# HSoumi/hybrid-als-twotower-recommender

Measured on NVIDIA B200. Metric: als_ratings_per_sec_per_sweep, higher is better.
Workload: dtype f32

## Files before the change

hybrid-als-twotower-recommender_b200/csrc/als_tc_common.cuh:

```cuda
#pragma once
#include <cuda_bf16.h>
#include <stdint.h>

#include "als_prep.cuh"
#include "common.cuh"

namespace hals {

__device__ __forceinline__ float4 lds128(uint32_t addr) {
  float4 v;
  asm volatile("ld.shared.v4.f32 {%0,%1,%2,%3}, [%4];\n" : "=f"(v.x), "=f"(v.y), "=f"(v.z), "=f"(v.w) : "r"(addr));
  return v;
}
__device__ __forceinline__ float lds32(uint32_t addr) {
  float v;
  asm volatile("ld.shared.f32 %0, [%1];\n" : "=f"(v) : "r"(addr));
  return v;
}
__device__ __forceinline__ void sts128(uint32_t addr, float a, float b, float c, float d) {
  asm volatile("st.shared.v4.f32 [%0], {%1,%2,%3,%4};\n" ::"r"(addr), "f"(a), "f"(b), "f"(c), "f"(d) : "memory");
}
__device__ __forceinline__ void sts32(uint32_t addr, float a) {
  asm volatile("st.shared.f32 [%0], %1;\n" ::"r"(addr), "f"(a) : "memory");
}

typedef unsigned long long f32x2;
__device__ __forceinline__ f32x2 pack2(float lo, float hi) {
  f32x2 r;
  asm("mov.b64 %0, {%1, %2};\n" : "=l"(r) : "f"(lo), "f"(hi));
  return r;
}
__device__ __forceinline__ float lo2(f32x2 v) { return __uint_as_float((uint32_t)v); }
__device__ __forceinline__ float hi2(f32x2 v) { return __uint_as_float((uint32_t)(v >> 32)); }
__device__ __forceinline__ f32x2 ffma2(f32x2 a, f32x2 b, f32x2 c) {
  f32x2 d;
  asm("fma.rn.f32x2 %0, %1, %2, %3;\n" : "=l"(d) : "l"(a), "l"(b), "l"(c));
  return d;
}
__device__ __forceinline__ void lds128x2(uint32_t addr, f32x2& p0, f32x2& p1) {
  asm volatile("ld.shared.v2.b64 {%0,%1}, [%2];\n" : "=l"(p0), "=l"(p1) : "r"(addr));
}
__device__ __forceinline__ f32x2 lds64x2(uint32_t addr) {
  f32x2 p;
  asm volatile("ld.shared.b64 %0, [%1];\n" : "=l"(p) : "r"(addr));
  return p;
}
__device__ __forceinline__ void sts128x2(uint32_t addr, f32x2 p0, f32x2 p1) {
  asm volatile("st.shared.v2.b64 [%0], {%1,%2};\n" ::"r"(addr), "l"(p0), "l"(p1) : "memory");
}

__device__ __forceinline__ void sts128x2_if(bool pred, uint32_t addr, f32x2 p0, f32x2 p1) {
  asm volatile("{\n\t.reg .pred p;\n\tsetp.ne.b32 p, %3, 0;\n\t@p st.shared.v2.b64 [%0], {%1,%2};\n\t}\n"
               ::"r"(addr), "l"(p0), "l"(p1), "r"((uint32_t)pred) : "memory");
}
__device__ __forceinline__ void sts32_if(bool pred, uint32_t addr, float a) {
  asm volatile("{\n\t.reg .pred p;\n\tsetp.ne.b32 p, %2, 0;\n\t@p st.shared.f32 [%0], %1;\n\t}\n"
               ::"r"(addr), "f"(a), "r"((uint32_t)pred) : "memory");
}

__device__ __forceinline__ void bar_sync_64(int id) { asm volatile("bar.sync %0, 64;\n" ::"r"(id) : "memory"); }


__device__ __forceinline__ void bar_arrive_n(int id, int nthreads) {
  asm volatile("bar.arrive %0, %1;\n" ::"r"(id), "r"(nthreads) : "memory");
}
__device__ __forceinline__ void bar_sync_n(int id, int nthreads) {
  asm volatile("bar.sync %0, %1;\n" ::"r"(id), "r"(nthreads) : "memory");
}

int als_launch_reduce_solve128(const float* slots, float* dst, float reg, const hals_als_plan* plan, void* dst_hl,
                               const float* gram, cudaStream_t st);

}
```

hybrid-als-twotower-recommender_b200/csrc/als_ws64.cu:

```cuda
#include <cuda_bf16.h>

#include <cstdlib>

#include "als_ws_common.cuh"

namespace hals {
namespace ws64 {
using namespace ws;

constexpr int K = 64;
constexpr int kStageBytes = stage_bytes(K);
#ifndef HALS_WS_STAGES
#define HALS_WS_STAGES 10
#endif
constexpr int kStages = HALS_WS_STAGES;
constexpr int kAcc = 4, kAccCols = 128;
constexpr int kSlots = 2;
constexpr int kLd = 68;
constexpr int kSlotBytes = 2 * 64 * kLd * 4 + 512;
constexpr int kSolvers = 9;
constexpr int kScratchBytes = 1536;
constexpr int kN = 80;
constexpr int kThreads = 512;
constexpr int kWarpSolver = 0, kWarpGather = 9, kWarpMma = 11, kWarpDrain = 12;
static_assert(kStages % 2 == 0, "the two gather warps own alternate stages");
static_assert(kWarpSolver + kSolvers == kWarpGather && kWarpDrain + 4 == kThreads / 32 && kWarpDrain % 4 == 0, "role map");

struct Bars {
  uint64_t st_full[kStages], st_free[kStages];
  uint64_t st_scaled[kStages];
  uint64_t acc_full[kAcc], acc_free[kAcc];
  uint64_t sol_full[kSolvers];
  uint64_t slot_free[kSlots];
};

__device__ __forceinline__ float sel4(float a, float b, float c, float d, int i) {
  return i == 0 ? a : i == 1 ? b : i == 2 ? c : d;
}

__device__ __noinline__ void gather_role(uint32_t stages, Bars* bars, uint8_t* gscratch, const Range* rg,
                                         const int32_t* __restrict__ colidx, const uint32_t* __restrict__ vals_hl,
                                         const float* __restrict__ vals_sc, const uint8_t* __restrict__ src_hl, int zero_row,
                                         const int64_t* __restrict__ chunk_pos, const int32_t* __restrict__ chunk_cnt,
                                         int gw, int lane) {
  const int t_sub = lane >> 4, piece = lane & 15;
  const uint32_t ring = umma::smem_u32(gscratch);
  const uint32_t mpos = ring + 2 * kBurst * 128;
  const uint32_t mcnt = mpos + 2 * kBurst * 8;
  const int64_t k_hi = rg->chunk_hi;
  int64_t kw = rg->chunk_lo + gw;
  auto load_window = [&](int64_t& p, int& c) {
    const int64_t k = kw + 2 * lane;
    p = 0; c = 0;
    if (k < k_hi) { p = __ldg(chunk_pos + k); c = __ldg(chunk_cnt + k); }
    kw += 64;
  };
  int64_t wpos, npos;
  int wcnt, ncnt;
  load_window(wpos, wcnt);
  load_window(npos, ncnt);
  int wb = 0;
  int ci[kBurst];
  auto fill = [&](int buf) {
    if (lane >= wb * kBurst && lane < (wb + 1) * kBurst) {
      const uint32_t e = (uint32_t)(buf * kBurst + lane - wb * kBurst);
      asm volatile("st.shared.b64 [%0], %1;\n" ::"r"(mpos + e * 8u), "l"(wpos) : "memory");
      asm volatile("st.shared.b32 [%0], %1;\n" ::"r"(mcnt + e * 4u), "r"(wcnt) : "memory");
    }
#pragma unroll
    for (int c = 0; c < kBurst; ++c) {
      const int64_t pos = __shfl_sync(0xffffffffu, wpos, wb * kBurst + c);
      const int cnt = __shfl_sync(0xffffffffu, wcnt, wb * kBurst + c);
      ci[c] = lane < cnt ? __ldg(colidx + pos + lane) : zero_row;
    }
    if (++wb == 32 / kBurst) {
      wb = 0;
      wpos = npos; wcnt = ncnt;
      load_window(npos, ncnt);
    }
  };
  auto stash = [&](int buf) {
#pragma unroll
    for (int c = 0; c < kBurst; ++c)
      sts32(ring + (uint32_t)((buf * kBurst + c) * 32 + (lane & 1) * 16 + (lane >> 1)) * 4u, __int_as_float(ci[c]));
    __syncwarp();
  };

  const uint32_t blk_off = piece < 8 ? 0u : (uint32_t)kBlk;
  uint32_t dsto[4];
#pragma unroll
  for (int i = 0; i < 4; ++i) {
    const int t = t_sub + 2 * i;
    dsto[i] = blk_off + (uint32_t)t * kRowBytes + (uint32_t)(((piece & 7) ^ (t & 7)) << 4);
  }
  const uint64_t srcb = reinterpret_cast<uint64_t>(src_hl) + (uint64_t)piece * 16u;
  const uint32_t rdst = 2 * kBlk + (uint32_t)lane * kRowBytes + (uint32_t)((lane & 7) << 4);
  const uint32_t sdst = 2 * kBlk + (uint32_t)lane * kRowBytes + (uint32_t)((7 ^ (lane & 7)) << 4);
  uint32_t g = 0, s = (uint32_t)gw, u = 0;
#ifdef HALS_WS_PROFILE
  long long w_free = 0, t_iss = 0, t_fill = 0;
#endif
  fill(0);
  stash(0);
  fill(1);
  for (int buf = 0;; buf ^= 1) {
    bool done = false;
#pragma unroll 1
    for (int c = 0; c < kBurst; ++c) {
      int cnt;
      asm volatile("ld.shared.b32 %0, [%1];\n" : "=r"(cnt) : "r"(mcnt + (uint32_t)(buf * kBurst + c) * 4u));
      if (cnt <= 0) { done = true; break; }
      int64_t pos;
      asm volatile("ld.shared.b64 %0, [%1];\n" : "=l"(pos) : "r"(mpos + (uint32_t)(buf * kBurst + c) * 8u));
      const uint32_t ir = ring + (uint32_t)((buf * kBurst + c) * 32 + t_sub * 16) * 4u;
      const float4 c0 = lds128(ir), c1 = lds128(ir + 16), c2 = lds128(ir + 32), c3 = lds128(ir + 48);
      if (u > 0) { WS_T0(); umma::mbar_wait(&bars->st_free[s], (u - 1) & 1); WS_ACC(w_free); }
      WS_T0();
      const uint32_t st = stages + s * kStageBytes;
      const float colf[16] = {c0.x, c0.y, c0.z, c0.w, c1.x, c1.y, c1.z, c1.w, c2.x, c2.y, c2.z, c2.w, c3.x, c3.y, c3.z, c3.w};
#pragma unroll
      for (int i = 0; i < KC / 2; ++i) {
        uint64_t src;
        asm("mad.wide.u32 %0, %1, 256, %2;\n" : "=l"(src) : "r"((uint32_t)__float_as_int(colf[i])), "l"(srcb));
        cp_async16_raw(st + dsto[i & 3] + (uint32_t)(i >> 2) * (8 * kRowBytes), src);
      }
      {
        const bool ok = lane < cnt;
        const uint32_t* rp = vals_hl + pos + (ok ? lane : 0);
        asm volatile("cp.async.ca.shared.global [%0], [%1], 4, %2;\n" ::"r"(st + rdst), "l"(rp), "r"(ok ? 4 : 0) : "memory");
        if (vals_sc != nullptr) {
          const float* sp = vals_sc + pos + (ok ? lane : 0);
          asm volatile("cp.async.ca.shared.global [%0], [%1], 4, %2;\n" ::"r"(st + sdst), "l"(sp), "r"(ok ? 4 : 0) : "memory");
        }
      }
      cp_async_mbar_arrive_noinc(&bars->st_full[s]);
      WS_ACC(t_iss);
      ++g;
      s += 2;
      if (s >= (uint32_t)kStages) { s -= kStages; ++u; }
    }
    if (done) break;
    WS_T0();
    stash(buf ^ 1);
    fill(buf);
    WS_ACC(t_fill);
  }
#ifdef HALS_WS_PROFILE
  if (lane == 0 && blockIdx.x == 1) printf("G%d: chunks %u wait_free %lld issue %lld fill %lld\n", gw, g, w_free, t_iss, t_fill);
#endif
}

__device__ __noinline__ void scaler_role(uint32_t stages, Bars* bars, const Range* rg, int lane) {
  scale_stages<K, kStages>(stages, bars, rg, lane);
}

__device__ __noinline__ void mma_role(uint32_t sbase, uint32_t tmem, Bars* bars, const Range* rg,
                                      const int32_t* __restrict__ chunk_cnt, bool scaled, int lane) {
  constexpr uint32_t idesc = umma::make_instr_desc(umma::kFmtBF16, true, true, 128, kN);
  uint64_t* const ready = scaled ? bars->st_scaled : bars->st_full;
  const int64_t k_lo = rg->chunk_lo, k_hi = rg->chunk_hi;
  uint32_t s = 0, su = 0, b = 0, bu = 0;
  bool first = true;
#ifdef HALS_WS_PROFILE
  long long w_acc = 0, w_full = 0, t_issue = 0;
#endif
  int wc = 0, nc = 0;
  if (k_lo + lane < k_hi) wc = __ldg(chunk_cnt + k_lo + lane);
  if (k_lo + 32 + lane < k_hi) nc = __ldg(chunk_cnt + k_lo + 32 + lane);
  const bool leader = elect_one();
  const uint64_t ad0 = umma::make_smem_desc(sbase, kBlk, 1024, umma::kSwizzle128B);
  const uint64_t bd0 = umma::make_smem_desc(sbase, 2 * kBlk, 1024, umma::kSwizzle128B);
  for (int64_t kb = k_lo; kb < k_hi; kb += 32) {
    const int nk = (int)(k_hi - kb < 32 ? k_hi - kb : 32);
    for (int i = 0; i < nk; ++i) {
      const int cnt = __shfl_sync(0xffffffffu, wc, i);
      if (leader) {
        if (first) {
          if (bu > 0) { WS_T0(); umma::mbar_wait(&bars->acc_free[b], (bu - 1) & 1); WS_ACC(w_acc); }
          umma::fence_after_sync();
        }
        { WS_T0(); umma::mbar_wait(&ready[s], su & 1); WS_ACC(w_full); }
        WS_T0();
        const uint32_t td = tmem + b * kAccCols;
        const uint64_t so = (uint64_t)((s * kStageBytes) >> 4);
#pragma unroll
        for (int ks = 0; ks < KC / 16; ++ks)
          umma::mma_bf16(td, ad0 + so + (uint64_t)(ks * 2048 >> 4), bd0 + so + (uint64_t)(ks * 2048 >> 4), idesc,
                         !(first && ks == 0));
        umma::commit(&bars->st_free[s]);
        if (cnt <= KC) umma::commit(&bars->acc_full[b]);
        WS_ACC(t_issue);
      }
      __syncwarp();
      first = cnt <= KC;
      if (first) { if (++b == (uint32_t)kAcc) { b = 0; ++bu; } }
      if (++s == (uint32_t)kStages) { s = 0; ++su; }
    }
    wc = nc;
    nc = 0;
    if (kb + 64 + lane < k_hi) nc = __ldg(chunk_cnt + kb + 64 + lane);
  }
#ifdef HALS_WS_PROFILE
  if (blockIdx.x == 1 && leader) printf("M: wait_acc_free %lld wait_stage_full %lld issue %lld\n", w_acc, w_full, t_issue);
#endif
}

__device__ __noinline__ void drain_role(uint32_t slots, uint32_t tmem, Bars* bars, const Range* rg, int nsolv, int tid) {
  const int warp = tid >> 5;
  const int64_t n_rows = rg->item_hi - rg->item_lo;
  uint32_t b = 0, bu = 0, sl = 0, slu = 0, sv = 0;
#ifdef HALS_WS_PROFILE
  long long w_acc = 0, w_slot = 0, t_ld = 0;
#endif
  for (int64_t it = 0; it < n_rows; ++it) {
    { WS_T0(); umma::mbar_wait(&bars->acc_full[b], bu & 1); WS_ACC(w_acc); }
    umma::fence_after_sync();
    const uint32_t ta = tmem + b * kAccCols + ((uint32_t)(warp * 32) << 16);
    float a[64], e[16];
    {
      WS_T0();
      umma::tmem_ld32(ta, a);
      umma::tmem_ld32(ta + 32, a + 32);
      umma::tmem_ld16(ta + 64, e);
      WS_ACC(t_ld);
    }
    umma::fence_before_sync();
    umma::mbar_arrive(&bars->acc_free[b]);
    if (slu > 0) { WS_T0(); umma::mbar_wait(&bars->slot_free[sl], (slu - 1) & 1); WS_ACC(w_slot); }
    const uint32_t sb = slots + sl * kSlotBytes;
    const int m = tid & 63;
    const uint32_t rowp = sb + (tid < 64 ? 0u : (uint32_t)(64 * kLd * 4)) + (uint32_t)m * (kLd * 4);
#pragma unroll
    for (int n = 0; n < 64; n += 4) sts128(rowp + n * 4, a[n], a[n + 1], a[n + 2], a[n + 3]);
    const uint32_t bp = sb + 2 * 64 * kLd * 4;
    if (tid < 64) sts32(bp + m * 4, e[0] + e[1]);
    else sts32(bp + 256 + m * 4, e[0]);
    umma::mbar_arrive(&bars->sol_full[sv]);
    if (++b == (uint32_t)kAcc) { b = 0; ++bu; }
    if (++sl == (uint32_t)kSlots) { sl = 0; ++slu; }
    if (++sv == (uint32_t)nsolv) sv = 0;
  }
#ifdef HALS_WS_PROFILE
  if (tid == 0 && blockIdx.x == 1) printf("D: wait_acc_full %lld tmem_ld %lld wait_slot_free %lld\n", w_acc, t_ld, w_slot);
#endif
}

template <int JR>
__device__ __forceinline__ void elim_block(f32x2 (&R)[36], f32x2& bb2, const uint32_t P, const uint32_t Y,
                                           const uint32_t DI, const int ti, const int tj, const int lane) {
  const uint32_t oW = (uint32_t)ti * 16u;
  const uint32_t oL = (uint32_t)(tj & 3) * 16u + (uint32_t)(tj >> 2) * 4u;
  const uint32_t oB = oW + (uint32_t)(tj >> 1) * 64u + (uint32_t)(tj & 1) * 8u;
  auto publish = [&](uint32_t Pn, bool own) {
    if (JR & 1) sts64_if(own, Pn + oW + (JR >> 1) * 64 + 8, R[tri(JR, JR)]);
#pragma unroll
    for (int q = (JR + 1) & ~1; q < 8; q += 2) sts128x2_if(own, Pn + oW + (q >> 1) * 64, R[tri(q, JR)], R[tri(q + 1, JR)]);
  };
  {
    publish(P, tj == 0);
    sts32_if(ti == 0 && tj == JR, Y + (uint32_t)(8 * JR) * 4u, lo2(bb2));
    sts32_if(lane == 0, DI + (uint32_t)(8 * JR) * 4u, -rcp_fast(lo2(R[tri(JR, JR)])));
    __syncwarp();
  }
  const bool below = tj > JR;
#pragma unroll 1
  for (int jm = 0; jm < 8; ++jm) {
    const int j = 8 * JR + jm;
    const uint32_t Pj = P + ((uint32_t)(jm & 1) << 8);
    f32x2 w[8];
    float l[8];
    if (JR & 1) w[JR] = lds64x2(Pj + oW + (JR >> 1) * 64 + 8);
#pragma unroll
    for (int q = (JR + 1) & ~1; q < 8; q += 2) lds128x2(Pj + oW + (q >> 1) * 64, w[q], w[q + 1]);
    const float ninv = lds32(DI + (uint32_t)j * 4u);
#pragma unroll
    for (int c = JR; c < 8; ++c) l[c] = lds32(Pj + oL + (c >> 1) * 64 + (c & 1) * 8);
    const float zj = lds32(Y + (uint32_t)j * 4u);
    const f32x2 wb = lds64x2(Pj + oB);
    const f32x2 ninv2 = pack2(ninv, ninv);
    const float lj = tj > jm ? l[JR] : 0.f;
    const f32x2 lj2 = pack2(lj, lj);
    w[JR] = fmul2(w[JR], ninv2);
    R[tri(JR, JR)] = ffma2(w[JR], lj2, R[tri(JR, JR)]);
    const int jn = jm + 1;
    const float ninv_n = -rcp_fast((jn & 4) ? hi2(R[tri(JR, JR)]) : lo2(R[tri(JR, JR)]));
#pragma unroll
    for (int q = JR + 1; q < 8; ++q) {
      w[q] = fmul2(w[q], ninv2);
      R[tri(q, JR)] = ffma2(w[q], lj2, R[tri(q, JR)]);
    }
    {
      const bool on = tj == JR;
      const bool act_lo = below || (on && ti > jm), act_hi = below || (on && ti + 4 > jm);
      const f32x2 mb = fmul2(wb, ninv2);
      bb2 = ffma2(pack2(act_lo ? lo2(mb) : 0.f, act_hi ? hi2(mb) : 0.f), pack2(zj, zj), bb2);
    }
    {
      const uint32_t Pn = P + ((uint32_t)(jn & 1) << 8);
      const bool own = (tj == jn);
      publish(Pn, own);
      sts32_if(tj == JR && ti == (jn & 3) && jn < 8, Y + (uint32_t)(j + 1) * 4u, (jn & 4) ? hi2(bb2) : lo2(bb2));
      sts32_if(own && ti == (jn & 3), DI + (uint32_t)(j + 1) * 4u, ninv_n);
      __syncwarp();
    }
#pragma unroll
    for (int c = JR + 1; c < 8; ++c) {
      const f32x2 l2 = pack2(l[c], l[c]);
#pragma unroll
      for (int q = c; q < 8; ++q) R[tri(q, c)] = ffma2(w[q], l2, R[tri(q, c)]);
    }
  }
}

template <int JR>
__device__ __forceinline__ void back_block(const f32x2 (&R)[36], f32x2 (&x2)[8], const uint32_t Y, const uint32_t DI,
                                           const uint32_t T, const uint32_t RH, const int ti, const int tj,
                                           const int lane, float& out0, float& out1) {
  f32x2 acc0 = 0ull, acc1 = 0ull;
#pragma unroll
  for (int q = JR + 1; q < 8; ++q) {
    if ((q - JR) & 1) acc0 = ffma2(R[tri(q, JR)], x2[q], acc0);
    else acc1 = ffma2(R[tri(q, JR)], x2[q], acc1);
  }
  float ext = (lo2(acc0) + hi2(acc0)) + (lo2(acc1) + hi2(acc1));
  ext += __shfl_xor_sync(0xffffffffu, ext, 8);
  ext += __shfl_xor_sync(0xffffffffu, ext, 16);
  const float rh = lds32(Y + (uint32_t)(8 * JR + tj) * 4u) - ext;
  sts32(T + (uint32_t)(ti * 8 + tj) * 4u, lo2(R[tri(JR, JR)]));
  sts32(T + (uint32_t)((ti + 4) * 8 + tj) * 4u, hi2(R[tri(JR, JR)]));
  sts32_if(ti == 0, RH + (uint32_t)tj * 4u, rh);
  __syncwarp();
  float r[8], di[8], xb[8];
  {
    const float4 a = lds128(RH), b = lds128(RH + 16);
    r[0] = a.x; r[1] = a.y; r[2] = a.z; r[3] = a.w; r[4] = b.x; r[5] = b.y; r[6] = b.z; r[7] = b.w;
    const float4 c = lds128(DI + (uint32_t)(8 * JR) * 4u), d = lds128(DI + (uint32_t)(8 * JR) * 4u + 16);
    di[0] = c.x; di[1] = c.y; di[2] = c.z; di[3] = c.w; di[4] = d.x; di[5] = d.y; di[6] = d.z; di[7] = d.w;
  }
#pragma unroll
  for (int e = 7; e >= 0; --e) {
    xb[e] = -r[e] * di[e];
    if (e > 0) {
      float t[8];
      const float4 a = lds128(T + (uint32_t)(e * 8) * 4u);
      t[0] = a.x; t[1] = a.y; t[2] = a.z; t[3] = a.w;
      if (e > 4) {
        const float4 b = lds128(T + (uint32_t)(e * 8 + 4) * 4u);
        t[4] = b.x; t[5] = b.y; t[6] = b.z; t[7] = b.w;
      }
#pragma unroll
      for (int c = 0; c < e; ++c) r[c] = fmaf(-t[c], xb[e], r[c]);
    }
  }
  __syncwarp();
  x2[JR] = pack2(sel4(xb[0], xb[1], xb[2], xb[3], ti), sel4(xb[4], xb[5], xb[6], xb[7], ti));
  if ((lane >> 2) == JR) {
    const int e2 = lane & 3;
    out0 = sel4(xb[0], xb[2], xb[4], xb[6], e2);
    out1 = sel4(xb[1], xb[3], xb[5], xb[7], e2);
  }
}

__device__ __forceinline__ void eliminate(f32x2 (&R)[36], f32x2& bb2, const uint32_t P, const uint32_t Y, const uint32_t DI,
                                          int ti, int tj, int lane) {
  elim_block<0>(R, bb2, P, Y, DI, ti, tj, lane);
  elim_block<1>(R, bb2, P, Y, DI, ti, tj, lane);
  elim_block<2>(R, bb2, P, Y, DI, ti, tj, lane);
  elim_block<3>(R, bb2, P, Y, DI, ti, tj, lane);
  elim_block<4>(R, bb2, P, Y, DI, ti, tj, lane);
  elim_block<5>(R, bb2, P, Y, DI, ti, tj, lane);
  elim_block<6>(R, bb2, P, Y, DI, ti, tj, lane);
  elim_block<7>(R, bb2, P, Y, DI, ti, tj, lane);
  __syncwarp();
}
__device__ __forceinline__ void back_store(const f32x2 (&R)[36], const uint32_t Y, const uint32_t DI, const uint32_t T,
                                           const uint32_t RH, int ti, int tj, int lane, float* __restrict__ dst,
                                           __nv_bfloat16* __restrict__ dst_hl, int row) {
  f32x2 x2[8];
#pragma unroll
  for (int q = 0; q < 8; ++q) x2[q] = 0ull;
  float out0 = 0.f, out1 = 0.f;
  back_block<7>(R, x2, Y, DI, T, RH, ti, tj, lane, out0, out1);
  back_block<6>(R, x2, Y, DI, T, RH, ti, tj, lane, out0, out1);
  back_block<5>(R, x2, Y, DI, T, RH, ti, tj, lane, out0, out1);
  back_block<4>(R, x2, Y, DI, T, RH, ti, tj, lane, out0, out1);
  back_block<3>(R, x2, Y, DI, T, RH, ti, tj, lane, out0, out1);
  back_block<2>(R, x2, Y, DI, T, RH, ti, tj, lane, out0, out1);
  back_block<1>(R, x2, Y, DI, T, RH, ti, tj, lane, out0, out1);
  back_block<0>(R, x2, Y, DI, T, RH, ti, tj, lane, out0, out1);
  *reinterpret_cast<float2*>(dst + (int64_t)row * K + 2 * lane) = make_float2(out0, out1);
  if (dst_hl) {
    const __nv_bfloat162 h = __floats2bfloat162_rn(out0, out1);
    const __nv_bfloat162 l = __floats2bfloat162_rn(out0 - __low2float(h), out1 - __high2float(h));
    __nv_bfloat162* o = reinterpret_cast<__nv_bfloat162*>(dst_hl + (int64_t)row * (2 * K));
    o[lane] = h;
    o[K / 2 + lane] = l;
  }
}

__device__ __noinline__ void solver_role(uint32_t slots, uint32_t scratch, Bars* bars, float* __restrict__ dst,
                                         __nv_bfloat16* __restrict__ dst_hl, float* __restrict__ workspace, float reg,
                                         const int32_t* __restrict__ item_row, const int32_t* __restrict__ item_len,
                                         const int32_t* __restrict__ item_slot, const float* __restrict__ gram_tiles,
                                         const Range* rg, int nsolv, int w, int lane) {
  const int ti = lane >> 3, tj = lane & 7;
  const uint32_t P = scratch, Y = P + 512, DI = Y + 256, T = DI + 256, RH = T + 256;
  const int64_t n_items = rg->item_hi;
#ifdef HALS_WS_PROFILE
  long long w_slot = 0, t_load = 0, t_elim = 0, t_back = 0;
  int n_solved = 0;
#endif
  int64_t it = rg->item_lo + w;
  int row_n = 0, len_n = 0, slot_n = -1;
  if (it < n_items) { row_n = __ldg(item_row + it); len_n = __ldg(item_len + it); slot_n = __ldg(item_slot + it); }
  uint32_t mine = 0;
  for (uint32_t i = (uint32_t)w; it < n_items; i += nsolv, it += nsolv, ++mine) {
    const int row = row_n, len = len_n, wslot = slot_n;
    {
      const int64_t nx = it + nsolv;
      if (nx < n_items) { row_n = __ldg(item_row + nx); len_n = __ldg(item_len + nx); slot_n = __ldg(item_slot + nx); }
    }
    const uint32_t sl = i % kSlots;
    { WS_T0(); umma::mbar_wait(&bars->sol_full[w], mine & 1); WS_ACC(w_slot); }
    const uint32_t S1 = slots + sl * kSlotBytes, S2 = S1 + 64 * kLd * 4, B1 = S2 + 64 * kLd * 4, B2 = B1 + 256;
    if (wslot >= 0) {
      float* W = workspace + (size_t)wslot * ((size_t)K * K + K + 4);
      for (int e = lane; e < K * K; e += 32) {
        const int m = e >> 6, n = e & 63;
        W[e] = lds32(S1 + (uint32_t)(m * kLd + n) * 4u) + lds32(S2 + (uint32_t)(m * kLd + n) * 4u) +
               lds32(S2 + (uint32_t)(n * kLd + m) * 4u);
      }
      W[K * K + lane] = lds32(B1 + lane * 4) + lds32(B2 + lane * 4);
      W[K * K + 32 + lane] = lds32(B1 + (32 + lane) * 4) + lds32(B2 + (32 + lane) * 4);
      if (lane == 0) W[K * K + K] = (float)len;
      __syncwarp();
      if (lane == 0) umma::mbar_arrive(&bars->slot_free[sl]);
      continue;
    }
    f32x2 R[36];
    f32x2 bb2;
    {
      WS_T0();
      const float lam = reg * (float)len;
      const uint32_t p1 = S1 + (uint32_t)(ti * kLd + tj) * 4u, p2 = S2 + (uint32_t)(ti * kLd + tj) * 4u;
      const uint32_t pt = S2 + (uint32_t)(tj * kLd + ti) * 4u;
#pragma unroll
      for (int q = 0; q < 8; ++q) {
#pragma unroll
        for (int c = 0; c <= q; ++c) {
          float v[2];
#pragma unroll
          for (int h = 0; h < 2; ++h) {
            const uint32_t mn = (uint32_t)((8 * q + 4 * h) * kLd + 8 * c) * 4u, nm = (uint32_t)(8 * c * kLd + 8 * q + 4 * h) * 4u;
            v[h] = lds32(p1 + mn) + lds32(p2 + mn) + lds32(pt + nm);
            if (q == c) v[h] += (ti + 4 * h == tj) ? lam : 0.f;
          }
          R[tri(q, c)] = pack2(v[0], v[1]);
        }
      }
      if (gram_tiles != nullptr) {
        const float4* gp = reinterpret_cast<const float4*>(gram_tiles) + lane * 18;
#pragma unroll
        for (int i = 0; i < 18; ++i) {
          const float4 g = __ldg(gp + i);
          R[2 * i] = ffma2(pack2(g.x, g.y), pack2(1.f, 1.f), R[2 * i]);
          R[2 * i + 1] = ffma2(pack2(g.z, g.w), pack2(1.f, 1.f), R[2 * i + 1]);
        }
      }
      const uint32_t ob = (uint32_t)(ti + 8 * tj) * 4u;
      bb2 = pack2(lds32(B1 + ob) + lds32(B2 + ob), lds32(B1 + ob + 16) + lds32(B2 + ob + 16));
      __syncwarp();
      if (lane == 0) umma::mbar_arrive(&bars->slot_free[sl]);
      WS_ACC(t_load);
    }
    {
      WS_T0();
      eliminate(R, bb2, P, Y, DI, ti, tj, lane);
      WS_ACC(t_elim);
    }
    {
      WS_T0();
      back_store(R, Y, DI, T, RH, ti, tj, lane, dst, dst_hl, row);
      WS_ACC(t_back);
    }
#ifdef HALS_WS_PROFILE
    ++n_solved;
#endif
  }
#ifdef HALS_WS_PROFILE
  if (lane == 0 && blockIdx.x == 1)
    printf("S%d: solved %d wait_slot %lld load %lld elim %lld back %lld\n", w, n_solved, w_slot, t_load, t_elim, t_back);
#endif
}

__global__ void __launch_bounds__(kThreads, 1)
als_ws64_kernel(const int32_t* __restrict__ colidx, const uint32_t* __restrict__ vals_hl,
                const float* __restrict__ vals_sc, const float* __restrict__ gram_tiles,
                const __nv_bfloat16* __restrict__ src_hl, float* __restrict__ dst, float reg,
                const int32_t* __restrict__ item_row, const int32_t* __restrict__ item_len,
                const int32_t* __restrict__ item_slot, const int64_t* __restrict__ item_chunk0,
                const int64_t* __restrict__ item_cost0, const int64_t* __restrict__ chunk_pos,
                const int32_t* __restrict__ chunk_cnt, int64_t n_items, int zero_row, float* __restrict__ workspace,
                __nv_bfloat16* __restrict__ dst_hl) {
  extern __shared__ uint8_t smem_dyn[];
  __shared__ Bars bars;
  __shared__ Range range;
  __shared__ uint32_t tmem_slot;
  uint8_t* base = reinterpret_cast<uint8_t*>((reinterpret_cast<uintptr_t>(smem_dyn) + 1023) & ~uintptr_t(1023));
  const int tid = threadIdx.x, warp = tid >> 5, lane = tid & 31;
  if (warp == kWarpDrain) umma::tmem_alloc(&tmem_slot, kAcc * kAccCols);
  if (tid == 32) {
    for (int s = 0; s < kStages; ++s) {
      umma::mbar_init(&bars.st_full[s], 32);
      umma::mbar_init(&bars.st_free[s], 1);
      umma::mbar_init(&bars.st_scaled[s], 1);
    }
    for (int b = 0; b < kAcc; ++b) { umma::mbar_init(&bars.acc_full[b], 1); umma::mbar_init(&bars.acc_free[b], 128); }
    for (int s = 0; s < kSlots; ++s) umma::mbar_init(&bars.slot_free[s], 1);
    for (int s = 0; s < kSolvers; ++s) umma::mbar_init(&bars.sol_full[s], 128);
    umma::mbar_fence_init();
  }
  if (tid < 2) cta_range(&range, item_cost0, item_chunk0, n_items, tid);
  zero_r_blocks<K, kStages, kThreads>(base, tid);
  umma::fence_proxy_async();
  umma::fence_before_sync();
  __syncthreads();
  umma::fence_after_sync();
  const uint32_t tmem = tmem_slot;
  const uint32_t sbase = umma::smem_u32(base);
#ifdef HALS_WS_PROFILE
  const long long t_cta0 = clock64();
#endif
  const uint32_t slots = sbase + kStages * kStageBytes;
  const uint32_t scratch = slots + kSlots * kSlotBytes;
  uint8_t* gscratch = base + kStages * kStageBytes + kSlots * kSlotBytes + kSolvers * kScratchBytes;

  const bool implicit = vals_sc != nullptr;
  const int nsolv = implicit ? kSolvers - 1 : kSolvers;
  if (warp >= kWarpDrain) {
    drain_role(slots, tmem, &bars, &range, nsolv, tid - kWarpDrain * 32);
  } else if (warp >= kWarpGather && warp < kWarpMma) {
    gather_role(sbase, &bars, gscratch + (warp - kWarpGather) * kGatherScratch, &range, colidx, vals_hl, vals_sc,
                reinterpret_cast<const uint8_t*>(src_hl), zero_row, chunk_pos, chunk_cnt, warp - kWarpGather, lane);
  } else if (warp == kWarpMma) {
    mma_role(sbase, tmem, &bars, &range, chunk_cnt, implicit, lane);
  } else if (warp - kWarpSolver < nsolv) {
    solver_role(slots, scratch + (uint32_t)(warp - kWarpSolver) * kScratchBytes, &bars, dst, dst_hl, workspace, reg, item_row,
                item_len, item_slot, gram_tiles, &range, nsolv, warp - kWarpSolver, lane);
  } else {
    scaler_role(sbase, &bars, &range, lane);
  }
#ifdef HALS_WS_PROFILE
  const long long t_role = clock64() - t_cta0;
#endif
  umma::fence_before_sync();
  __syncthreads();
#ifdef HALS_WS_PROFILE
  if (lane == 0 && (warp == kWarpDrain || warp == kWarpGather || warp == kWarpMma || warp == kWarpSolver))
    printf("C %d w%d role %lld cta %lld\n", (int)blockIdx.x, warp, t_role, clock64() - t_cta0);
#endif
  if (warp == kWarpDrain) umma::tmem_dealloc(tmem, kAcc * kAccCols);
}

__global__ void __launch_bounds__(128)
als_reduce_solve64_warp_kernel(const float* __restrict__ workspace, float* __restrict__ dst,
                               __nv_bfloat16* __restrict__ dst_hl, float reg, const int32_t* __restrict__ long_row,
                               const int32_t* __restrict__ long_slot0, const int32_t* __restrict__ long_nseg,
                               const float* __restrict__ gram) {
  constexpr int SF = K * K + K + 4;
  __shared__ __align__(16) float sA[SF];
  __shared__ __align__(16) uint8_t sScratch[kScratchBytes];
  const int tid = threadIdx.x, lane = tid & 31;
  const int row = long_row[blockIdx.x];
  const int s0 = long_slot0[blockIdx.x], ns = long_nseg[blockIdx.x];
  const int stride = slot_final_stride(ns);
  for (int e = tid * 4; e < SF; e += 128 * 4) {
    float4 acc = make_float4(0.f, 0.f, 0.f, 0.f);
    for (int q = 0; q < ns; q += stride) {
      const float4 v = *reinterpret_cast<const float4*>(workspace + (size_t)(s0 + q) * SF + e);
      acc.x += v.x; acc.y += v.y; acc.z += v.z; acc.w += v.w;
    }
    *reinterpret_cast<float4*>(sA + e) = acc;
  }
  __syncthreads();
  if (tid >= 32) return;
  const int ti = lane >> 3, tj = lane & 7;
  const float lam = reg * sA[K * K + K];
  f32x2 R[36];
#pragma unroll
  for (int q = 0; q < 8; ++q) {
#pragma unroll
    for (int c = 0; c <= q; ++c) {
      float v[2];
#pragma unroll
      for (int h = 0; h < 2; ++h) {
        const int m = ti + 4 * h + 8 * q, n = tj + 8 * c;
        v[h] = sA[m * K + n] + (m == n ? lam : 0.f) + (gram != nullptr ? __ldg(gram + m * K + n) : 0.f);
      }
      R[tri(q, c)] = pack2(v[0], v[1]);
    }
  }
  f32x2 bb2 = pack2(sA[K * K + ti + 8 * tj], sA[K * K + ti + 4 + 8 * tj]);
  const uint32_t P = umma::smem_u32(sScratch), Y = P + 512, DI = Y + 256, T = DI + 256, RH = T + 256;
  eliminate(R, bb2, P, Y, DI, ti, tj, lane);
  back_store(R, Y, DI, T, RH, ti, tj, lane, dst, dst_hl, row);
}

}

__global__ void gram_to_tiles64_kernel(const float* __restrict__ G, float* __restrict__ tiles) {
  const int lane = threadIdx.x, ti = lane >> 3, tj = lane & 7;
  for (int q = 0; q < 8; ++q)
    for (int c = 0; c <= q; ++c)
      for (int h = 0; h < 2; ++h)
        tiles[lane * 72 + ws64::tri(q, c) * 2 + h] = G[(ti + 4 * h + 8 * q) * ws64::K + tj + 8 * c];
}

int als_half_step_ws64(const int32_t* colidx, const uint32_t* vals_hl, const float* src, int64_t n_src, float* dst,
                       float reg, const hals_als_plan* plan, float* slots, void* split_buf, void* dst_hl,
                       const float* gram, float* gram_tiles, cudaStream_t st) {
  using namespace ws64;
  __nv_bfloat16* hl = reinterpret_cast<__nv_bfloat16*>(split_buf);
  HALS_REQUIRE(n_src < (int64_t)1 << 31, "at most 2^31 - 1 source rows");
  if (src != nullptr) {
    if (int rc = als_launch_split_bf16(src, n_src, K, hl, st)) return rc;
    HALS_CUDA(cudaMemsetAsync(hl + (size_t)n_src * 2 * K, 0, 4 * K, st));
  }
  const size_t smem = (size_t)kStages * kStageBytes + (size_t)kSlots * kSlotBytes + (size_t)kSolvers * kScratchBytes +
                      2 * kGatherScratch + 1024;
  static_assert(kStages * kStageBytes + kSlots * kSlotBytes + kSolvers * kScratchBytes + 2 * kGatherScratch + 1024 <= 227 * 1024 - 1024,
                "shared memory budget");
  HALS_CUDA(cudaFuncSetAttribute(als_ws64_kernel, cudaFuncAttributeMaxDynamicSharedMemorySize, (int)smem));
  const bool implicit = gram != nullptr;
  if (implicit) {
    HALS_REQUIRE(plan->vals_scale && plan->item_npos && gram_tiles, "implicit mode needs the plan's vals_scale / item_npos");
    gram_to_tiles64_kernel<<<1, 32, 0, st>>>(gram, gram_tiles);
    HALS_LAUNCH_CHECK();
  }
  int64_t grid = sm_count();
  if (grid > plan->n_items) grid = plan->n_items;
  als_ws64_kernel<<<(unsigned)grid, kThreads, smem, st>>>(colidx, vals_hl, implicit ? plan->vals_scale : nullptr,
                                                         implicit ? gram_tiles : nullptr, hl, dst, reg, plan->item_row,
                                                         implicit ? plan->item_npos : plan->item_len, plan->item_slot, plan->item_chunk0, plan->item_cost0,
                                                         plan->chunk_pos, plan->chunk_cnt, plan->n_items, (int)n_src, slots,
                                                         reinterpret_cast<__nv_bfloat16*>(dst_hl));
  HALS_LAUNCH_CHECK();
  if (plan->n_long_rows > 0) {
    if (int rc = als_launch_slot_group_sum(slots, plan, K * K + K + 4, st)) return rc;
    als_reduce_solve64_warp_kernel<<<(unsigned)plan->n_long_rows, 128, 0, st>>>(
        slots, dst, reinterpret_cast<__nv_bfloat16*>(dst_hl), reg, plan->long_row, plan->long_slot0, plan->long_nseg, gram);
    HALS_LAUNCH_CHECK();
  }
  return 0;
}

}
```

hybrid-als-twotower-recommender_b200/csrc/als_ws_common.cuh:

```cuda
#pragma once
#include <cuda_bf16.h>

#include "als_common.cuh"
#include "als_tc_common.cuh"
#include "umma.cuh"

namespace hals {
namespace ws {

constexpr int KC = 32;
constexpr int kRowBytes = 128;
constexpr int kBlk = KC * kRowBytes;
__host__ __device__ constexpr int stage_bytes(int K) { return (K / 32 + 1) * kBlk; }

#ifdef HALS_WS_PROFILE
#define WS_T0() const long long t0__ = clock64()
#define WS_ACC(v) (v) += clock64() - t0__
#else
#define WS_T0() do { } while (0)
#define WS_ACC(v) do { } while (0)
#endif

__device__ __forceinline__ void sts64_if(bool pred, uint32_t addr, f32x2 p) {
  asm volatile("{\n\t.reg .pred p;\n\tsetp.ne.b32 p, %2, 0;\n\t@p st.shared.b64 [%0], %1;\n\t}\n"
               ::"r"(addr), "l"(p), "r"((uint32_t)pred) : "memory");
}
__device__ __forceinline__ void cp_async_mbar_arrive_noinc(uint64_t* mbar) {
  asm volatile("cp.async.mbarrier.arrive.noinc.shared::cta.b64 [%0];\n" ::"r"(umma::smem_u32(mbar)) : "memory");
}
__device__ __forceinline__ bool elect_one() {
  uint32_t p;
  asm volatile("{\n\t.reg .pred p;\n\telect.sync _|p, 0xffffffff;\n\tselp.u32 %0, 1, 0, p;\n\t}\n" : "=r"(p));
  return p != 0;
}
__device__ __forceinline__ f32x2 fmul2(f32x2 a, f32x2 b) { return ffma2(a, b, 0ull); }
__device__ __forceinline__ float rcp_fast(float d) {
  float r;
  asm("rcp.approx.ftz.f32 %0, %1;\n" : "=f"(r) : "f"(d));
  return r;
}
__host__ __device__ constexpr int tri(int q, int c) { return q * (q + 1) / 2 + c; }
__device__ __forceinline__ void cp_async16_raw(uint32_t smem_dst, uint64_t gsrc) {
  asm volatile("cp.async.cg.shared.global [%0], [%1], 16;\n" ::"r"(smem_dst), "l"(gsrc) : "memory");
}
__device__ __forceinline__ uint32_t cvt_bf16x2(float hi, float lo) {
  uint32_t d;
  asm("cvt.rn.bf16x2.f32 %0, %1, %2;\n" : "=r"(d) : "f"(hi), "f"(lo));
  return d;
}
__device__ __forceinline__ f32x2 unpack_bf16x2(uint32_t w) {
  return pack2(__uint_as_float(w << 16), __uint_as_float(w & 0xffff0000u));
}

struct Range {
  int64_t item_lo, item_hi, chunk_lo, chunk_hi;
};

__device__ __forceinline__ void cta_range(Range* range, const int64_t* __restrict__ item_cost0,
                                          const int64_t* __restrict__ item_chunk0, int64_t n_items, int tid) {
  const int64_t total = item_cost0[n_items];
  const int64_t bq = (int64_t)blockIdx.x + tid;
  const int64_t target = (total * bq + gridDim.x - 1) / gridDim.x;
  int64_t lo = 0, hi = n_items;
  while (lo < hi) {
    const int64_t mid = (lo + hi) >> 1;
    if (__ldg(item_cost0 + mid) < target) lo = mid + 1; else hi = mid;
  }
  if (bq == gridDim.x) lo = n_items;
  const int64_t ck = __ldg(item_chunk0 + lo);
  if (tid == 0) { range->item_lo = lo; range->chunk_lo = ck; } else { range->item_hi = lo; range->chunk_hi = ck; }
}

template <int K, int kStages, int kThreads>
__device__ __forceinline__ void zero_r_blocks(uint8_t* base, int tid) {
  for (int i = tid; i < kStages * (kBlk / 16); i += kThreads)
    *reinterpret_cast<uint4*>(base + (i / (kBlk / 16)) * stage_bytes(K) + (stage_bytes(K) - kBlk) + (i % (kBlk / 16)) * 16) =
        make_uint4(0u, 0u, 0u, 0u);
}

constexpr int kBurst = 8;
constexpr int kGatherScratch = 2 * kBurst * 32 * 4 + 2 * kBurst * 8 + 2 * kBurst * 4;

template <int K, int kStages, class Bars>
__device__ __forceinline__ void scale_stages(uint32_t stages, Bars* bars, const Range* rg, int lane) {
  const int64_t k_lo = rg->chunk_lo, k_hi = rg->chunk_hi;
  const uint32_t rowo = (uint32_t)lane * kRowBytes, x = (uint32_t)(lane & 7);
  const f32x2 one2 = pack2(1.f, 1.f), mone2 = pack2(-1.f, -1.f);
  uint32_t s = 0, su = 0;
  for (int64_t k = k_lo; k < k_hi; ++k) {
    umma::mbar_wait(&bars->st_full[s], su & 1);
    const uint32_t st = stages + s * stage_bytes(K);
    const float sc = lds32(st + stage_bytes(K) - kBlk + rowo + ((7u ^ x) << 4));
    const f32x2 sc2 = pack2(sc, sc);
#pragma unroll 2
    for (int i = 0; i < K / 8; ++i) {
      const uint32_t off = st + (uint32_t)(i >> 3) * kBlk + rowo + ((((uint32_t)i & 7u) ^ x) << 4);
      const float4 hv = lds128(off), lv = lds128(off + (K / 64) * kBlk);
      const uint32_t hw[4] = {__float_as_uint(hv.x), __float_as_uint(hv.y), __float_as_uint(hv.z), __float_as_uint(hv.w)};
      const uint32_t lw[4] = {__float_as_uint(lv.x), __float_as_uint(lv.y), __float_as_uint(lv.z), __float_as_uint(lv.w)};
      uint32_t oh[4], ol[4];
#pragma unroll
      for (int j = 0; j < 4; ++j) {
        const f32x2 y = ffma2(unpack_bf16x2(hw[j]), one2, unpack_bf16x2(lw[j]));
        const f32x2 v = fmul2(y, sc2);
        oh[j] = cvt_bf16x2(hi2(v), lo2(v));
        const f32x2 r = ffma2(unpack_bf16x2(oh[j]), mone2, v);
        ol[j] = cvt_bf16x2(hi2(r), lo2(r));
      }
      sts128(off, __uint_as_float(oh[0]), __uint_as_float(oh[1]), __uint_as_float(oh[2]), __uint_as_float(oh[3]));
      sts128(off + (K / 64) * kBlk, __uint_as_float(ol[0]), __uint_as_float(ol[1]), __uint_as_float(ol[2]), __uint_as_float(ol[3]));
    }
    umma::fence_proxy_async();
    __syncwarp();
    if (lane == 0) umma::mbar_arrive(&bars->st_scaled[s]);
    if (++s == (uint32_t)kStages) { s = 0; ++su; }
  }
}

}
}
```

Baseline: 6.213 billion.

## Restructure solver elimination with precomputed lane role masks and shared-memory args

Rewrites the per-column elimination step so each lane's predicates and addresses come from a precomputed role bitmask that is shifted each step, and the column buffer is flipped by XOR on address bit 8. Pivot reciprocals are stored interleaved next to the Y values and the sign is folded into the FMAs. Solver kernel arguments move into a shared-memory struct that is loaded on demand, and per-item metadata prefetching is dropped. Together these are meant to cut register pressure and integer or predicate work in the solver warps' inner loop. The cost is more complex, tightly coupled indexing and a new 512-byte alignment requirement on scratch.

After: 6.479 billion, median of 6. 1.04x the previous value.

```diff
diff --git a/hybrid-als-twotower-recommender_b200/csrc/als_tc_common.cuh b/hybrid-als-twotower-recommender_b200/csrc/als_tc_common.cuh
--- a/hybrid-als-twotower-recommender_b200/csrc/als_tc_common.cuh
+++ b/hybrid-als-twotower-recommender_b200/csrc/als_tc_common.cuh
@@ -49,13 +49,13 @@
   asm volatile("st.shared.v2.b64 [%0], {%1,%2};\n" ::"r"(addr), "l"(p0), "l"(p1) : "memory");
 }
 
-__device__ __forceinline__ void sts128x2_if(bool pred, uint32_t addr, f32x2 p0, f32x2 p1) {
+__device__ __forceinline__ void sts128x2_if(uint32_t pred, uint32_t addr, f32x2 p0, f32x2 p1) {
   asm volatile("{\n\t.reg .pred p;\n\tsetp.ne.b32 p, %3, 0;\n\t@p st.shared.v2.b64 [%0], {%1,%2};\n\t}\n"
-               ::"r"(addr), "l"(p0), "l"(p1), "r"((uint32_t)pred) : "memory");
+               ::"r"(addr), "l"(p0), "l"(p1), "r"(pred) : "memory");
 }
-__device__ __forceinline__ void sts32_if(bool pred, uint32_t addr, float a) {
+__device__ __forceinline__ void sts32_if(uint32_t pred, uint32_t addr, float a) {
   asm volatile("{\n\t.reg .pred p;\n\tsetp.ne.b32 p, %2, 0;\n\t@p st.shared.f32 [%0], %1;\n\t}\n"
-               ::"r"(addr), "f"(a), "r"((uint32_t)pred) : "memory");
+               ::"r"(addr), "f"(a), "r"(pred) : "memory");
 }
 
 __device__ __forceinline__ void bar_sync_64(int id) { asm volatile("bar.sync %0, 64;\n" ::"r"(id) : "memory"); }
diff --git a/hybrid-als-twotower-recommender_b200/csrc/als_ws64.cu b/hybrid-als-twotower-recommender_b200/csrc/als_ws64.cu
--- a/hybrid-als-twotower-recommender_b200/csrc/als_ws64.cu
+++ b/hybrid-als-twotower-recommender_b200/csrc/als_ws64.cu
@@ -25,6 +25,8 @@
 constexpr int kWarpSolver = 0, kWarpGather = 9, kWarpMma = 11, kWarpDrain = 12;
 static_assert(kStages % 2 == 0, "the two gather warps own alternate stages");
 static_assert(kWarpSolver + kSolvers == kWarpGather && kWarpDrain + 4 == kThreads / 32 && kWarpDrain % 4 == 0, "role map");
+static_assert(kStageBytes % 512 == 0 && kSlotBytes % 512 == 0 && kScratchBytes % 512 == 0,
+              "a solver's scratch is 512-byte aligned: its elimination steps flip the column buffer by bit 8");
 
 struct Bars {
   uint64_t st_full[kStages], st_free[kStages];
@@ -245,71 +247,99 @@
 #endif
 }
 
+struct Lane {
+  uint32_t pw, pl, pb;
+  uint32_t dsel;
+  uint32_t roles;
+};
+constexpr int kRoleLive = 0;
+constexpr int kRoleZ = 8;
+constexpr int kRoleOwn = 16;
+constexpr int kRoleZhi = 24;
+
+__device__ __forceinline__ Lane lane_setup(uint32_t P) {
+  uint32_t lane;
+  asm volatile("mov.u32 %0, %%laneid;\n" : "=r"(lane));
+  const uint32_t ti = lane >> 3, tj = lane & 7;
+  Lane L;
+  L.pw = P + ti * 16u;
+  L.pl = P + (tj & 3) * 16u + (tj >> 2) * 4u;
+  L.pb = L.pw + (tj >> 1) * 64u + (tj & 1) * 8u;
+  L.dsel = (tj & 4 ? 0x7654u : 0x3210u) | (ti == (tj & 3) ? 3u << kRoleOwn : 0u);
+  const uint32_t z = ti == 0 ? 0x08u : 0x11u << (ti - 1);
+  L.roles = (((1u << tj) - 1u) << kRoleLive) | (z << kRoleZ) | (((1u << tj) >> 1) << kRoleOwn) | (0xf8u << kRoleZhi);
+  return L;
+}
+
+__device__ __forceinline__ float sel_if(uint32_t pred, float a, float b) {
+  float r;
+  asm("{\n\t.reg .pred p;\n\tsetp.ne.b32 p, %1, 0;\n\tselp.f32 %0, %2, %3, p;\n\t}\n" : "=f"(r) : "r"(pred), "f"(a), "f"(b));
+  return r;
+}
+
 template <int JR>
-__device__ __forceinline__ void elim_block(f32x2 (&R)[36], f32x2& bb2, const uint32_t P, const uint32_t Y,
-                                           const uint32_t DI, const int ti, const int tj, const int lane) {
-  const uint32_t oW = (uint32_t)ti * 16u;
-  const uint32_t oL = (uint32_t)(tj & 3) * 16u + (uint32_t)(tj >> 2) * 4u;
-  const uint32_t oB = oW + (uint32_t)(tj >> 1) * 64u + (uint32_t)(tj & 1) * 8u;
-  auto publish = [&](uint32_t Pn, bool own) {
-    if (JR & 1) sts64_if(own, Pn + oW + (JR >> 1) * 64 + 8, R[tri(JR, JR)]);
-#pragma unroll
-    for (int q = (JR + 1) & ~1; q < 8; q += 2) sts128x2_if(own, Pn + oW + (q >> 1) * 64, R[tri(q, JR)], R[tri(q + 1, JR)]);
-  };
+__device__ __forceinline__ void publish_column(const f32x2 (&R)[36], uint32_t pw, uint32_t own) {
+  if (JR & 1) sts64_if(own, pw + (JR >> 1) * 64 + 8, R[tri(JR, JR)]);
+#pragma unroll
+  for (int q = (JR + 1) & ~1; q < 8; q += 2) sts128x2_if(own, pw + (q >> 1) * 64, R[tri(q, JR)], R[tri(q + 1, JR)]);
+}
+
+template <int JR>
+__device__ __forceinline__ void elim_step(f32x2 (&R)[36], f32x2& bb2, const Lane& L, const uint32_t yj, const uint32_t roles) {
+  f32x2 w[8];
+  float l[8];
+  if (JR & 1) w[JR] = lds64x2(L.pw + (JR >> 1) * 64 + 8);
+#pragma unroll
+  for (int q = (JR + 1) & ~1; q < 8; q += 2) lds128x2(L.pw + (q >> 1) * 64, w[q], w[q + 1]);
+  const float dinv = lds32(yj + 256);
+#pragma unroll
+  for (int c = JR; c < 8; ++c) l[c] = lds32(L.pl + (c >> 1) * 64 + (c & 1) * 8);
+  const float zj = lds32(yj);
+  const f32x2 wb = lds64x2(L.pb);
+  const f32x2 dinv2 = pack2(dinv, dinv);
+  const float lj = sel_if(roles & (1u << kRoleLive), l[JR], 0.f);
+  w[JR] = fmul2(w[JR], dinv2);
+  R[tri(JR, JR)] = ffma2(w[JR], pack2(-lj, -lj), R[tri(JR, JR)]);
+  const float dinv_n = rcp_fast(__uint_as_float(
+      __byte_perm(__float_as_uint(lo2(R[tri(JR, JR)])), __float_as_uint(hi2(R[tri(JR, JR)])), L.dsel)));
+#pragma unroll
+  for (int q = JR + 1; q < 8; ++q) {
+    w[q] = fmul2(w[q], dinv2);
+    R[tri(q, JR)] = ffma2(w[q], pack2(-lj, -lj), R[tri(q, JR)]);
+  }
+  bb2 = ffma2(fmul2(wb, dinv2), pack2(-zj, -zj), bb2);
   {
-    publish(P, tj == 0);
-    sts32_if(ti == 0 && tj == JR, Y + (uint32_t)(8 * JR) * 4u, lo2(bb2));
-    sts32_if(lane == 0, DI + (uint32_t)(8 * JR) * 4u, -rcp_fast(lo2(R[tri(JR, JR)])));
+    const uint32_t own = roles & (1u << kRoleOwn);
+    publish_column<JR>(R, L.pw ^ 256u, own);
+    sts32_if(roles & (1u << kRoleZ), yj + 4, sel_if(roles & (1u << kRoleZhi), hi2(bb2), lo2(bb2)));
+    sts32_if(own & L.dsel, yj + 256 + 4, dinv_n);
     __syncwarp();
   }
-  const bool below = tj > JR;
+#pragma unroll
+  for (int c = JR + 1; c < 8; ++c) {
+#pragma unroll
+    for (int q = c; q < 8; ++q) R[tri(q, c)] = ffma2(w[q], pack2(-l[c], -l[c]), R[tri(q, c)]);
+  }
+}
+
+template <int JR>
+__device__ __forceinline__ void elim_block(f32x2 (&R)[36], f32x2& bb2, Lane& L, uint32_t& yj) {
+  const bool zblk = (L.roles & (JR ? 3u << (JR - 1) : 1u)) == (JR ? 1u << (JR - 1) : 0u);
+  uint32_t roles = zblk ? L.roles : L.roles & ~(0xffu << kRoleZ);
+  {
+    const bool own0 = (L.roles & (1u << kRoleLive)) == 0;
+    publish_column<JR>(R, L.pw, own0);
+    sts32_if(roles & (1u << (kRoleZ + 3)), yj, lo2(bb2));
+    sts32_if(own0 && (L.dsel & (1u << kRoleOwn)), yj + 256, rcp_fast(lo2(R[tri(JR, JR)])));
+    __syncwarp();
+  }
 #pragma unroll 1
-  for (int jm = 0; jm < 8; ++jm) {
-    const int j = 8 * JR + jm;
-    const uint32_t Pj = P + ((uint32_t)(jm & 1) << 8);
-    f32x2 w[8];
-    float l[8];
-    if (JR & 1) w[JR] = lds64x2(Pj + oW + (JR >> 1) * 64 + 8);
-#pragma unroll
-    for (int q = (JR + 1) & ~1; q < 8; q += 2) lds128x2(Pj + oW + (q >> 1) * 64, w[q], w[q + 1]);
-    const float ninv = lds32(DI + (uint32_t)j * 4u);
-#pragma unroll
-    for (int c = JR; c < 8; ++c) l[c] = lds32(Pj + oL + (c >> 1) * 64 + (c & 1) * 8);
-    const float zj = lds32(Y + (uint32_t)j * 4u);
-    const f32x2 wb = lds64x2(Pj + oB);
-    const f32x2 ninv2 = pack2(ninv, ninv);
-    const float lj = tj > jm ? l[JR] : 0.f;
-    const f32x2 lj2 = pack2(lj, lj);
-    w[JR] = fmul2(w[JR], ninv2);
-    R[tri(JR, JR)] = ffma2(w[JR], lj2, R[tri(JR, JR)]);
-    const int jn = jm + 1;
-    const float ninv_n = -rcp_fast((jn & 4) ? hi2(R[tri(JR, JR)]) : lo2(R[tri(JR, JR)]));
-#pragma unroll
-    for (int q = JR + 1; q < 8; ++q) {
-      w[q] = fmul2(w[q], ninv2);
-      R[tri(q, JR)] = ffma2(w[q], lj2, R[tri(q, JR)]);
-    }
-    {
-      const bool on = tj == JR;
-      const bool act_lo = below || (on && ti > jm), act_hi = below || (on && ti + 4 > jm);
-      const f32x2 mb = fmul2(wb, ninv2);
-      bb2 = ffma2(pack2(act_lo ? lo2(mb) : 0.f, act_hi ? hi2(mb) : 0.f), pack2(zj, zj), bb2);
-    }
-    {
-      const uint32_t Pn = P + ((uint32_t)(jn & 1) << 8);
-      const bool own = (tj == jn);
-      publish(Pn, own);
-      sts32_if(tj == JR && ti == (jn & 3) && jn < 8, Y + (uint32_t)(j + 1) * 4u, (jn & 4) ? hi2(bb2) : lo2(bb2));
-      sts32_if(own && ti == (jn & 3), DI + (uint32_t)(j + 1) * 4u, ninv_n);
-      __syncwarp();
-    }
-#pragma unroll
-    for (int c = JR + 1; c < 8; ++c) {
-      const f32x2 l2 = pack2(l[c], l[c]);
-#pragma unroll
-      for (int q = c; q < 8; ++q) R[tri(q, c)] = ffma2(w[q], l2, R[tri(q, c)]);
-    }
-  }
+  do {
+    elim_step<JR>(R, bb2, L, yj, roles);
+    L.pw ^= 256u; L.pl ^= 256u; L.pb ^= 256u;
+    yj += 4;
+    roles >>= 1;
+  } while (roles >= 1u << kRoleZhi);
 }
 
 template <int JR>
@@ -339,7 +369,7 @@
   }
 #pragma unroll
   for (int e = 7; e >= 0; --e) {
-    xb[e] = -r[e] * di[e];
+    xb[e] = r[e] * di[e];
     if (e > 0) {
       float t[8];
       const float4 a = lds128(T + (uint32_t)(e * 8) * 4u);
@@ -361,16 +391,17 @@
   }
 }
 
-__device__ __forceinline__ void eliminate(f32x2 (&R)[36], f32x2& bb2, const uint32_t P, const uint32_t Y, const uint32_t DI,
-                                          int ti, int tj, int lane) {
-  elim_block<0>(R, bb2, P, Y, DI, ti, tj, lane);
-  elim_block<1>(R, bb2, P, Y, DI, ti, tj, lane);
-  elim_block<2>(R, bb2, P, Y, DI, ti, tj, lane);
-  elim_block<3>(R, bb2, P, Y, DI, ti, tj, lane);
-  elim_block<4>(R, bb2, P, Y, DI, ti, tj, lane);
-  elim_block<5>(R, bb2, P, Y, DI, ti, tj, lane);
-  elim_block<6>(R, bb2, P, Y, DI, ti, tj, lane);
-  elim_block<7>(R, bb2, P, Y, DI, ti, tj, lane);
+__device__ __forceinline__ void eliminate(f32x2 (&R)[36], f32x2& bb2, const uint32_t P, const uint32_t Y) {
+  Lane L = lane_setup(P);
+  uint32_t yj = Y;
+  elim_block<0>(R, bb2, L, yj);
+  elim_block<1>(R, bb2, L, yj);
+  elim_block<2>(R, bb2, L, yj);
+  elim_block<3>(R, bb2, L, yj);
+  elim_block<4>(R, bb2, L, yj);
+  elim_block<5>(R, bb2, L, yj);
+  elim_block<6>(R, bb2, L, yj);
+  elim_block<7>(R, bb2, L, yj);
   __syncwarp();
 }
 __device__ __forceinline__ void back_store(const f32x2 (&R)[36], const uint32_t Y, const uint32_t DI, const uint32_t T,
@@ -398,33 +429,43 @@
   }
 }
 
-__device__ __noinline__ void solver_role(uint32_t slots, uint32_t scratch, Bars* bars, float* __restrict__ dst,
-                                         __nv_bfloat16* __restrict__ dst_hl, float* __restrict__ workspace, float reg,
-                                         const int32_t* __restrict__ item_row, const int32_t* __restrict__ item_len,
-                                         const int32_t* __restrict__ item_slot, const float* __restrict__ gram_tiles,
+struct SolverArgs {
+  float* dst;
+  __nv_bfloat16* dst_hl;
+  float* workspace;
+  const float* gram_tiles;
+  const int32_t* item_row;
+  const int32_t* item_len;
+  const int32_t* item_slot;
+  float reg;
+};
+template <class T>
+__device__ __forceinline__ T* ld_arg(T* const& v) {
+  uint64_t r;
+  asm volatile("ld.shared.u64 %0, [%1];\n" : "=l"(r) : "r"(umma::smem_u32(&v)));
+  return reinterpret_cast<T*>(r);
+}
+__device__ __forceinline__ float ld_arg(const float& v) { return lds32(umma::smem_u32(&v)); }
+
+__device__ __noinline__ void solver_role(uint32_t slots, uint32_t scratch, Bars* bars, const SolverArgs* args,
                                          const Range* rg, int nsolv, int w, int lane) {
   const int ti = lane >> 3, tj = lane & 7;
   const uint32_t P = scratch, Y = P + 512, DI = Y + 256, T = DI + 256, RH = T + 256;
-  const int64_t n_items = rg->item_hi;
+  const uint32_t n_items = (uint32_t)(rg->item_hi - rg->item_lo);
 #ifdef HALS_WS_PROFILE
   long long w_slot = 0, t_load = 0, t_elim = 0, t_back = 0;
   int n_solved = 0;
 #endif
-  int64_t it = rg->item_lo + w;
-  int row_n = 0, len_n = 0, slot_n = -1;
-  if (it < n_items) { row_n = __ldg(item_row + it); len_n = __ldg(item_len + it); slot_n = __ldg(item_slot + it); }
-  uint32_t mine = 0;
-  for (uint32_t i = (uint32_t)w; it < n_items; i += nsolv, it += nsolv, ++mine) {
-    const int row = row_n, len = len_n, wslot = slot_n;
-    {
-      const int64_t nx = it + nsolv;
-      if (nx < n_items) { row_n = __ldg(item_row + nx); len_n = __ldg(item_len + nx); slot_n = __ldg(item_slot + nx); }
-    }
+  for (uint32_t mine = 0;; ++mine) {
+    const uint32_t i = (uint32_t)w + mine * (uint32_t)nsolv;
+    if (i >= n_items) break;
+    const int64_t it = rg->item_lo + i;
+    const int len = __ldg(ld_arg(args->item_len) + it), wslot = __ldg(ld_arg(args->item_slot) + it);
     const uint32_t sl = i % kSlots;
     { WS_T0(); umma::mbar_wait(&bars->sol_full[w], mine & 1); WS_ACC(w_slot); }
     const uint32_t S1 = slots + sl * kSlotBytes, S2 = S1 + 64 * kLd * 4, B1 = S2 + 64 * kLd * 4, B2 = B1 + 256;
     if (wslot >= 0) {
-      float* W = workspace + (size_t)wslot * ((size_t)K * K + K + 4);
+      float* W = ld_arg(args->workspace) + (size_t)wslot * ((size_t)K * K + K + 4);
       for (int e = lane; e < K * K; e += 32) {
         const int m = e >> 6, n = e & 63;
         W[e] = lds32(S1 + (uint32_t)(m * kLd + n) * 4u) + lds32(S2 + (uint32_t)(m * kLd + n) * 4u) +
@@ -441,7 +482,7 @@
     f32x2 bb2;
     {
       WS_T0();
-      const float lam = reg * (float)len;
+      const float lam = ld_arg(args->reg) * (float)len;
       const uint32_t p1 = S1 + (uint32_t)(ti * kLd + tj) * 4u, p2 = S2 + (uint32_t)(ti * kLd + tj) * 4u;
       const uint32_t pt = S2 + (uint32_t)(tj * kLd + ti) * 4u;
 #pragma unroll
@@ -458,6 +499,7 @@
           R[tri(q, c)] = pack2(v[0], v[1]);
         }
       }
+      const float* gram_tiles = ld_arg(args->gram_tiles);
       if (gram_tiles != nullptr) {
         const float4* gp = reinterpret_cast<const float4*>(gram_tiles) + lane * 18;
 #pragma unroll
@@ -475,12 +517,13 @@
     }
     {
       WS_T0();
-      eliminate(R, bb2, P, Y, DI, ti, tj, lane);
+      eliminate(R, bb2, P, Y);
       WS_ACC(t_elim);
     }
     {
       WS_T0();
-      back_store(R, Y, DI, T, RH, ti, tj, lane, dst, dst_hl, row);
+      const int row = __ldg(ld_arg(args->item_row) + it);
+      back_store(R, Y, DI, T, RH, ti, tj, lane, ld_arg(args->dst), ld_arg(args->dst_hl), row);
       WS_ACC(t_back);
     }
 #ifdef HALS_WS_PROFILE
@@ -505,6 +548,7 @@
   extern __shared__ uint8_t smem_dyn[];
   __shared__ Bars bars;
   __shared__ Range range;
+  __shared__ SolverArgs sargs;
   __shared__ uint32_t tmem_slot;
   uint8_t* base = reinterpret_cast<uint8_t*>((reinterpret_cast<uintptr_t>(smem_dyn) + 1023) & ~uintptr_t(1023));
   const int tid = threadIdx.x, warp = tid >> 5, lane = tid & 31;
@@ -521,6 +565,7 @@
     umma::mbar_fence_init();
   }
   if (tid < 2) cta_range(&range, item_cost0, item_chunk0, n_items, tid);
+  if (tid == 64) sargs = SolverArgs{dst, dst_hl, workspace, gram_tiles, item_row, item_len, item_slot, reg};
   zero_r_blocks<K, kStages, kThreads>(base, tid);
   umma::fence_proxy_async();
   umma::fence_before_sync();
@@ -545,8 +590,8 @@
   } else if (warp == kWarpMma) {
     mma_role(sbase, tmem, &bars, &range, chunk_cnt, implicit, lane);
   } else if (warp - kWarpSolver < nsolv) {
-    solver_role(slots, scratch + (uint32_t)(warp - kWarpSolver) * kScratchBytes, &bars, dst, dst_hl, workspace, reg, item_row,
-                item_len, item_slot, gram_tiles, &range, nsolv, warp - kWarpSolver, lane);
+    solver_role(slots, scratch + (uint32_t)(warp - kWarpSolver) * kScratchBytes, &bars, &sargs, &range, nsolv,
+                warp - kWarpSolver, lane);
   } else {
     scaler_role(sbase, &bars, &range, lane);
   }
@@ -569,7 +614,7 @@
                                const float* __restrict__ gram) {
   constexpr int SF = K * K + K + 4;
   __shared__ __align__(16) float sA[SF];
-  __shared__ __align__(16) uint8_t sScratch[kScratchBytes];
+  __shared__ __align__(512) uint8_t sScratch[kScratchBytes];
   const int tid = threadIdx.x, lane = tid & 31;
   const int row = long_row[blockIdx.x];
   const int s0 = long_slot0[blockIdx.x], ns = long_nseg[blockIdx.x];
@@ -602,7 +647,7 @@
   }
   f32x2 bb2 = pack2(sA[K * K + ti + 8 * tj], sA[K * K + ti + 4 + 8 * tj]);
   const uint32_t P = umma::smem_u32(sScratch), Y = P + 512, DI = Y + 256, T = DI + 256, RH = T + 256;
-  eliminate(R, bb2, P, Y, DI, ti, tj, lane);
+  eliminate(R, bb2, P, Y);
   back_store(R, Y, DI, T, RH, ti, tj, lane, dst, dst_hl, row);
 }
 
diff --git a/hybrid-als-twotower-recommender_b200/csrc/als_ws_common.cuh b/hybrid-als-twotower-recommender_b200/csrc/als_ws_common.cuh
--- a/hybrid-als-twotower-recommender_b200/csrc/als_ws_common.cuh
+++ b/hybrid-als-twotower-recommender_b200/csrc/als_ws_common.cuh
@@ -21,9 +21,9 @@
 #define WS_ACC(v) do { } while (0)
 #endif
 
-__device__ __forceinline__ void sts64_if(bool pred, uint32_t addr, f32x2 p) {
+__device__ __forceinline__ void sts64_if(uint32_t pred, uint32_t addr, f32x2 p) {
   asm volatile("{\n\t.reg .pred p;\n\tsetp.ne.b32 p, %2, 0;\n\t@p st.shared.b64 [%0], %1;\n\t}\n"
-               ::"r"(addr), "l"(p), "r"((uint32_t)pred) : "memory");
+               ::"r"(addr), "l"(p), "r"(pred) : "memory");
 }
 __device__ __forceinline__ void cp_async_mbar_arrive_noinc(uint64_t* mbar) {
   asm volatile("cp.async.mbarrier.arrive.noinc.shared::cta.b64 [%0];\n" ::"r"(umma::smem_u32(mbar)) : "memory");
```
